# saitejasrivilli/movie-recommender-demo

Hardware: AMD Instinct MI355X
Metric: end-to-end recs/sec (1M ads d=256, top-500->10) (higher is better)
Workload: dtype f32 (f16x3 emulation: 2 fp16 planes per operand, 3 fp16-MFMA products per MAC, fp32 accumulate)

## Files before the change

movie-recommender-demo_amd/csrc/rowowner16_common.hpp:

```cpp
#pragma once
#include "x3_common.hpp"

namespace amdrec {
namespace x16 {

using x3::DBG, x3::f16x8, x3::lds_cfloat, x3::TARGET_EXP;

__device__ __forceinline__ f32x4 mfma(const f16x8& a, const f16x8& b, const f32x4& c) {
    return __builtin_amdgcn_mfma_f32_16x16x32_f16(a, b, c, 0, 0, 0);
}
__device__ __forceinline__ void group6(const f16x8 (&a)[4], const f16x8& bh, const f16x8& bl, f32x4& c0, f32x4& c1) {
    c0 = mfma(a[0], bl, c0);
    c1 = mfma(a[2], bl, c1);
    c0 = mfma(a[1], bh, c0);
    c1 = mfma(a[3], bh, c1);
    c0 = mfma(a[0], bh, c0);
    c1 = mfma(a[2], bh, c1);
}

__device__ __forceinline__ float reduce_max4(float v) {
    v = fmaxf(v, __shfl_xor(v, 16, 64));
    return fmaxf(v, __shfl_xor(v, 32, 64));
}
__device__ __forceinline__ float reduce_sum4(float v) {
    v += __shfl_xor(v, 16, 64);
    return v + __shfl_xor(v, 32, 64);
}

__device__ __forceinline__ void row_scale(const f32x4 (&x)[16], float& s, float& inv) {
    float m = 0.f;
#pragma unroll
    for (int t = 0; t < 16; ++t)
#pragma unroll
        for (int r = 0; r < 4; ++r) m = fmaxf(m, __builtin_fabsf(x[t][r]));
    m = reduce_max4(m);
    int eb = (int)((__float_as_uint(m) >> 23) & 0xffu);
    eb = eb < 87 ? 87 : (eb > 250 ? 250 : eb);
    s = __uint_as_float((uint32_t)(127 + TARGET_EXP + 127 - eb) << 23);
    inv = __uint_as_float((uint32_t)(eb - TARGET_EXP) << 23);
}

__device__ __forceinline__ void split8(const f32x4& a, const f32x4& b, float s, f16x8& h, f16x8& l) {
#pragma unroll
    for (int j = 0; j < 8; ++j) {
        const float v = (j < 4 ? a[j & 3] : b[j & 3]) * s;
        const _Float16 hh = (_Float16)v;
        h[j] = hh;
        l[j] = (_Float16)(v - (float)hh);
    }
}

__device__ __forceinline__ f32x4 param4(lds_cfloat* pb, int off, int tile) {
    return *reinterpret_cast<const __attribute__((address_space(3))) f32x4*>(pb + off + 16 * tile);
}

template <bool WITH_X>
__device__ __forceinline__ void prepare(const f32x4 (&x)[16], float s, lds_cfloat* pb, int bias, float scale,
                                        f16x8 (&xh)[8], f16x8 (&xl)[8], f32x4 (&acc)[16]) {
#pragma unroll
    for (int ks = 0; ks < 8; ++ks) {
        split8(x[2 * ks], x[2 * ks + 1], s, xh[ks], xl[ks]);
#pragma unroll
        for (int t = 2 * ks; t < 2 * ks + 2; ++t) {
            const f32x4 b = param4(pb, bias, t);
#pragma unroll
            for (int r = 0; r < 4; ++r) acc[t][r] = ((WITH_X ? x[t][r] : 0.f) + b[r]) * scale;
        }
    }
}

__device__ __forceinline__ float layer_norm(f32x4 (&y)[16], lds_cfloat* pb, int gamma, int beta, float eps) {
    float s = 0.f;
#pragma unroll
    for (int t = 0; t < 16; ++t)
#pragma unroll
        for (int r = 0; r < 4; ++r) s += y[t][r];
    const float mean = reduce_sum4(s) * (1.0f / 256.0f);
    float q = 0.f;
#pragma unroll
    for (int t = 0; t < 16; ++t)
#pragma unroll
        for (int r = 0; r < 4; ++r) {
            const float d = y[t][r] - mean;
            q += d * d;
        }
    const float rstd = 1.0f / sqrtf(reduce_sum4(q) * (1.0f / 256.0f) + eps);
#pragma unroll
    for (int t = 0; t < 16; ++t) {
        const f32x4 ga = param4(pb, gamma, t), be = param4(pb, beta, t);
#pragma unroll
        for (int r = 0; r < 4; ++r) y[t][r] = (y[t][r] - mean) * rstd * ga[r] + be[r];
    }
    return rstd;
}

__device__ __forceinline__ void layer_norm_scaled(const f32x4 (&acc)[16], float un, f32x4 (&y)[16], lds_cfloat* pb, int gamma,
                                                  int beta, float eps) {
    float s = 0.f;
#pragma unroll
    for (int t = 0; t < 16; ++t)
#pragma unroll
        for (int r = 0; r < 4; ++r) s += acc[t][r];
    const float mean = reduce_sum4(s) * un * (1.0f / 256.0f);
    float q = 0.f;
#pragma unroll
    for (int t = 0; t < 16; ++t)
#pragma unroll
        for (int r = 0; r < 4; ++r) {
            const float d = __builtin_fmaf(acc[t][r], un, -mean);
            y[t][r] = d;
            q += d * d;
        }
    const float rstd = 1.0f / sqrtf(reduce_sum4(q) * (1.0f / 256.0f) + eps);
#pragma unroll
    for (int t = 0; t < 16; ++t) {
        const f32x4 ga = param4(pb, gamma, t), be = param4(pb, beta, t);
#pragma unroll
        for (int r = 0; r < 4; ++r) y[t][r] = y[t][r] * rstd * ga[r] + be[r];
    }
}

__device__ __forceinline__ void hidden_planes(const f32x4& a0, const f32x4& a1, float c, float lim, f16x8& hh, f16x8& hl) {
    if (DBG & 8) {
        asm volatile("" : "+v"(hh), "+v"(hl) : "v"(a0), "v"(a1));
        return;
    }
    f32x4 t0, t1;
#pragma unroll
    for (int r = 0; r < 4; ++r) {
        t0[r] = __builtin_amdgcn_fmed3f(a0[r], 0.f, lim);
        t1[r] = __builtin_amdgcn_fmed3f(a1[r], 0.f, lim);
    }
    split8(t0, t1, c, hh, hl);
}
__device__ __forceinline__ void init_pair(f32x4& a0, f32x4& a1, lds_cfloat* pb, int bias, int tile0, float scale) {
    const f32x4 b0 = param4(pb, bias, tile0), b1 = param4(pb, bias, tile0 + 1);
#pragma unroll
    for (int r = 0; r < 4; ++r) {
        a0[r] = b0[r] * scale;
        a1[r] = b1[r] * scale;
    }
}

__device__ __forceinline__ void load_rows(f32x4 (&x)[16], const float* row_ptr, int g) {
#pragma unroll
    for (int t = 0; t < 16; ++t) x[t] = *reinterpret_cast<const f32x4*>(row_ptr + 16 * t + 4 * g);
}
__device__ __forceinline__ void add_rows(f32x4 (&x)[16], const float* row_ptr, int g) {
#pragma unroll
    for (int t = 0; t < 16; ++t) {
        const f32x4 v = *reinterpret_cast<const f32x4*>(row_ptr + 16 * t + 4 * g);
#pragma unroll
        for (int r = 0; r < 4; ++r) x[t][r] += v[r];
    }
}
__device__ __forceinline__ void store_rows(const f32x4 (&x)[16], float* row_ptr, int g) {
#pragma unroll
    for (int t = 0; t < 16; ++t) *reinterpret_cast<f32x4*>(row_ptr + 16 * t + 4 * g) = x[t];
}

}
}
```

movie-recommender-demo_amd/csrc/rowowner16_impl.hpp:

```cpp

#pragma clang diagnostic push
#pragma clang diagnostic ignored "-Wuninitialized-const-reference"
namespace amdrec {
namespace AMDREC_X3B_NAMESPACE {

using x3::CHUNK_BYTES, x3::CHUNK_FRAGS, x3::DBG, x3::f16x8, x3::FRAG_BYTES, x3::Input, x3::lds_byte, x3::lds_cfloat, x3::Phase,
    x3::Program, x3::RING_BYTES;
using x16::add_rows, x16::group6, x16::hidden_planes, x16::init_pair, x16::layer_norm, x16::layer_norm_scaled, x16::load_rows,
    x16::param4, x16::prepare, x16::reduce_sum4, x16::row_scale, x16::split8, x16::store_rows;

#if !defined(AMDREC_X3B_WAVES) || !defined(AMDREC_X3B_NAMESPACE)
#error "include rowowner16.hpp, not this file"
#endif
constexpr int WAVES = AMDREC_X3B_WAVES, ROWS_PER_WAVE = 16, ROWS_PER_WG = WAVES * ROWS_PER_WAVE;
constexpr int DMA_PER_WAVE = CHUNK_FRAGS / WAVES;
constexpr bool PAIRED = WAVES == 8 && !(DBG & (256 | 512));
constexpr int NBUF = PAIRED ? x3::NBUF - 1 : x3::NBUF, DEPTH = NBUF - 3;
constexpr int PAIR_BYTES = CHUNK_BYTES / 4;
constexpr int DMA_GROUP = 1;

struct Ring {
    lds_byte* lds_dma;
    lds_byte* lds_rd;
    int issued, total;
    int slot;
    __amdgpu_buffer_rsrc_t rsrc;
    uint32_t voff, soff0;
    const lds_byte* cbase;
    unsigned long long t_wait, t_bar, t_dma;
    unsigned long long t_lds, t_cal;
    __device__ __forceinline__ void timed_landed(f16x8 (&f)[4]) {
        if (!(DBG & 32)) return;
        const unsigned long long a = __builtin_amdgcn_s_memtime();
        asm volatile("s_waitcnt lgkmcnt(0)" : "+v"(f[0]), "+v"(f[1]), "+v"(f[2]), "+v"(f[3]));
        const unsigned long long b = __builtin_amdgcn_s_memtime();
        t_lds += b - a;
    }

    template <int U>
    __device__ __forceinline__ void dma_pieces(lds_byte* dst, uint32_t so) {
        if constexpr (U < DMA_PER_WAVE) {
            __builtin_amdgcn_raw_ptr_buffer_load_lds(rsrc, (__attribute__((address_space(3))) void*)(dst + (U >> 2) * 4 * FRAG_BYTES),
                                                     16, voff, so + (U >> 2) * 4 * FRAG_BYTES, (U & 3) * FRAG_BYTES, 0);
            dma_pieces<U + 1>(dst, so);
        }
    }
    __device__ __forceinline__ void issue() {
        if (DBG & 1) { ++issued; return; }
        const int c = issued < total ? issued : total - 1;
        lds_byte* dst = lds_dma + (uint32_t)(issued % NBUF) * CHUNK_BYTES;
        const uint32_t so = __builtin_amdgcn_readfirstlane(soff0 + (uint32_t)c * CHUNK_BYTES);
        dma_pieces<0>(dst, so);
        ++issued;
    }
    template <int EXTRA = 0>
    __device__ __forceinline__ void certify_next() {
        if (DBG & 16) {
            const unsigned long long a = __builtin_amdgcn_s_memtime();
            asm volatile("s_waitcnt vmcnt(%0)" ::"n"(DMA_PER_WAVE * (DEPTH - 1)) : "memory");
            const unsigned long long b = __builtin_amdgcn_s_memtime();
            __builtin_amdgcn_s_barrier();
            const unsigned long long c = __builtin_amdgcn_s_memtime();
            const unsigned long long d = __builtin_amdgcn_s_memtime();
            t_wait += b - a; t_bar += c - b; t_dma += d - c;
            return;
        }
        if (!(DBG & 1)) asm volatile("s_waitcnt vmcnt(%0)" ::"n"(DMA_PER_WAVE * (DEPTH - 1) + EXTRA) : "memory");
        if (!(DBG & 2)) __builtin_amdgcn_s_barrier();
    }
    __device__ __forceinline__ void start(const unsigned char* stream, int total_chunks, lds_byte* lds, int wave, int lane) {
        voff = (uint32_t)lane * 16;
        soff0 = (uint32_t)wave * DMA_PER_WAVE * FRAG_BYTES;
        rsrc = __builtin_amdgcn_make_buffer_rsrc(const_cast<unsigned char*>(stream), 0, (uint32_t)total_chunks * CHUNK_BYTES,
                                                 0x00020000);
        lds_dma = lds + wave * DMA_PER_WAVE * FRAG_BYTES;
        lds_rd = lds + lane * 16;
        issued = 0;
        total = total_chunks;
        slot = -1;
        cbase = lds_rd;
        t_wait = t_bar = t_dma = t_lds = 0;
        t_cal = 0;
        if (DBG & 32) {
            const unsigned long long a = __builtin_amdgcn_s_memtime();
            asm volatile("s_waitcnt lgkmcnt(0)" ::: "memory");
            const unsigned long long b = __builtin_amdgcn_s_memtime();
            t_cal = b - a;
        }
#pragma unroll
        for (int c = 0; c < DEPTH + 1; ++c) issue();
        asm volatile("s_waitcnt vmcnt(%0)" ::"n"(DMA_PER_WAVE * DEPTH) : "memory");
        __builtin_amdgcn_s_barrier();
    }
    template <int EXTRA = 0>
    __device__ __forceinline__ void advance() {
        certify_next<EXTRA>();
        slot = slot + 1 == NBUF ? 0 : slot + 1;
        cbase = lds_rd + (uint32_t)slot * CHUNK_BYTES;
    }
    template <int G, bool HALF = false>
    __device__ __forceinline__ void frag4(f16x8 (&f)[4]) {
        static_assert(G >= 0 && G < 4 && CHUNK_FRAGS == 16, "four groups of four fragment sets per chunk");
        if ((DBG & 4) || ((DBG & 64) && G != 0) || ((DBG & 128) && (G & 1)) ||
            (HALF && (DBG & (256 | 512)) && (G & 1))) {
#pragma unroll
            for (int u = 0; u < 4; ++u) asm volatile("" : "+v"(f[u]));
        } else {
#pragma unroll
            for (int u = 0; u < 4; ++u)
                f[u] = *reinterpret_cast<const __attribute__((address_space(3))) f16x8*>(cbase + (4 * G + u) * FRAG_BYTES);
        }
    }
    template <int G, int EXTRA = 0, bool HALF = false>
    __device__ __forceinline__ void read4(f16x8 (&f)[4]) {
        if (G == 0) advance<EXTRA>();
        frag4<G, HALF>(f);
        if (G == DMA_GROUP) issue();
    }
    __device__ __forceinline__ void drain() { asm volatile("s_waitcnt vmcnt(0)" ::: "memory"); }
};

template <int I>
__device__ __forceinline__ void gemm256_groups(Ring& ring, f16x8 (&cur)[4], const f16x8 (&xh)[8], const f16x8 (&xl)[8],
                                               f32x4 (&acc)[16]) {
    constexpr int ks = I >> 3, tp = I & 7;
    f16x8 nxt[4];
    if constexpr (I < 63) ring.read4<(I + 1) & 3>(nxt);
    ring.timed_landed(cur);
    group6(cur, xh[ks], xl[ks], acc[2 * tp], acc[2 * tp + 1]);
    if constexpr (I < 63) gemm256_groups<I + 1>(ring, nxt, xh, xl, acc);
}
template <int I0>
__device__ __forceinline__ void gemm256_from(Ring& ring, const f16x8 (&xh)[8], const f16x8 (&xl)[8], f32x4 (&acc)[16]) {
    f16x8 cur[4];
    ring.read4<0>(cur);
    gemm256_groups<I0>(ring, cur, xh, xl, acc);
}

__device__ __forceinline__ void gemm256(Ring& ring, const f16x8 (&xh)[8], const f16x8 (&xl)[8], f32x4 (&acc)[16]) {
    gemm256_from<0>(ring, xh, xl, acc);
}
__device__ __forceinline__ void phase_attn_ln(Ring& ring, const Phase& P, f32x4 (&x)[16], lds_cfloat* pb) {
    float s, inv;
    row_scale(x, s, inv);
    f16x8 xh[8], xl[8];
    f32x4 acc[16];
    prepare<true>(x, s, pb, P.b1, s * P.sw1, xh, xl, acc);
    gemm256(ring, xh, xl, acc);
    layer_norm_scaled(acc, inv / P.sw1, x, pb, P.gamma, P.beta, P.ln_eps);
}

template <bool S1, bool S2, int GI, int EXTRA = 0, bool HALF = false>
__device__ __forceinline__ void ffn_groups(Ring& ring, f16x8 (&cur)[4], const f16x8 (&xh)[8], const f16x8 (&xl)[8],
                                           f32x4& a10, f32x4& a11, f32x4 (&acc2)[16], const f16x8& hh, const f16x8& hl) {
    constexpr int NG = (S1 ? 8 : 0) + (S2 ? 8 : 0);
    constexpr bool is1 = S1 && (!S2 || (GI & 1) == 0);
    constexpr int u = (S1 && S2) ? GI >> 1 : GI;
    f16x8 nxt[4];
    if constexpr (GI < NG - 1) ring.read4<(GI + 1) & 3, EXTRA, HALF>(nxt);
    ring.timed_landed(cur);
    if constexpr (is1) group6(cur, xh[u], xl[u], a10, a11);
    else group6(cur, hh, hl, acc2[2 * u], acc2[2 * u + 1]);
    if constexpr (GI < NG - 1) ffn_groups<S1, S2, GI + 1, EXTRA, HALF>(ring, nxt, xh, xl, a10, a11, acc2, hh, hl);
}

template <bool S1, bool S2, int EXTRA = 0, bool HALF = false>
__device__ __forceinline__ void ffn_step(Ring& ring, const f16x8 (&xh)[8], const f16x8 (&xl)[8], f32x4& a10, f32x4& a11,
                                         f32x4 (&acc2)[16], const f16x8& hh, const f16x8& hl) {
    f16x8 cur[4];
    ring.read4<0, EXTRA, HALF>(cur);
    ffn_groups<S1, S2, 0, EXTRA, HALF>(ring, cur, xh, xl, a10, a11, acc2, hh, hl);
}

__device__ __forceinline__ void ffn_hidden(const f32x4& a0, const f32x4& a1, float c, float lim, f16x8& hh, f16x8& hl) {
    if (DBG & 512) asm volatile("" : "+v"(hh), "+v"(hl) : "v"(a0), "v"(a1));
    else hidden_planes(a0, a1, c, lim, hh, hl);
}
__device__ __forceinline__ void phase_ffn_ln(Ring& ring, const Phase& P, f32x4 (&x)[16], lds_cfloat* pb) {
    float s, inv;
    row_scale(x, s, inv);
    f16x8 xh[8], xl[8];
    const float sh = x3::hidden_scale(fmaf(P.hn * 8192.0f, inv, P.hb));
    f32x4 acc2[16];
    prepare<true>(x, s, pb, P.b2, P.sw2 * sh, xh, xl, acc2);
    const float b1s = s * P.sw1, c1 = sh * inv / P.sw1, lim1 = 60000.f / c1;
    f32x4 a10, a11;
    f16x8 hh, hl;
    init_pair(a10, a11, pb, P.b1, 0, b1s);
    ffn_step<true, false, 0, true>(ring, xh, xl, a10, a11, acc2, hh, hl);
    for (int t = 1; t < P.n_steps; ++t) {
        ffn_hidden(a10, a11, c1, lim1, hh, hl);
        init_pair(a10, a11, pb, P.b1, 2 * t, b1s);
        ffn_step<true, true, 0, true>(ring, xh, xl, a10, a11, acc2, hh, hl);
    }
    ffn_hidden(a10, a11, c1, lim1, hh, hl);
    ffn_step<false, true, 0, true>(ring, xh, xl, a10, a11, acc2, hh, hl);
    layer_norm_scaled(acc2, 1.0f / (P.sw2 * sh), x, pb, P.gamma, P.beta, P.ln_eps);
}

template <int K, class V>
__device__ __forceinline__ void pair_put(lds_byte* box, const V& v) {
    static_assert(sizeof(V) == 16 && K >= 0 && K < PAIR_BYTES / FRAG_BYTES, "a 16-byte piece per lane");
    *reinterpret_cast<__attribute__((address_space(3))) V*>(box + K * FRAG_BYTES) = v;
}
template <int K, class V>
__device__ __forceinline__ void pair_get(const lds_byte* box, V& v) {
    static_assert(sizeof(V) == 16 && K >= 0 && K < PAIR_BYTES / FRAG_BYTES, "a 16-byte piece per lane");
    v = *reinterpret_cast<const __attribute__((address_space(3))) V*>(box + K * FRAG_BYTES);
}
__device__ __forceinline__ void pair_landed() { asm volatile("s_waitcnt lgkmcnt(0)" ::: "memory"); }
__device__ __forceinline__ void pair_sync() {
    pair_landed();
    __builtin_amdgcn_s_barrier();
}
__device__ __forceinline__ void group12(const f16x8 (&a)[4], const f16x8& bh0, const f16x8& bl0, const f16x8& bh1,
                                        const f16x8& bl1, f32x4& c00, f32x4& c01, f32x4& c10, f32x4& c11) {
    c00 = x16::mfma(a[0], bl0, c00);
    c01 = x16::mfma(a[2], bl0, c01);
    c10 = x16::mfma(a[0], bl1, c10);
    c11 = x16::mfma(a[2], bl1, c11);
    c00 = x16::mfma(a[1], bh0, c00);
    c01 = x16::mfma(a[3], bh0, c01);
    c10 = x16::mfma(a[1], bh1, c10);
    c11 = x16::mfma(a[3], bh1, c11);
    c00 = x16::mfma(a[0], bh0, c00);
    c01 = x16::mfma(a[2], bh0, c01);
    c10 = x16::mfma(a[0], bh1, c10);
    c11 = x16::mfma(a[2], bh1, c11);
}
template <int MODE, int J>
__device__ __forceinline__ void pair_read(Ring& ring, f16x8 (&f)[4]) {
    constexpr int G = MODE == 0 ? (J & 3) : 2 * (J & 1) + (MODE == 2 ? 1 : 0);
    if constexpr (G == (MODE == 2 ? 1 : 0)) ring.advance();
    ring.frag4<G>(f);
    if constexpr (G == (MODE == 1 ? 2 : DMA_GROUP)) ring.issue();
}
template <int MODE, int J>
__device__ __forceinline__ void pair_groups1(Ring& ring, f16x8 (&cur)[4], const f16x8 (&xh)[2][8], const f16x8 (&xl)[2][8],
                                             f32x4 (&a)[2][2]) {
    f16x8 nxt[4];
    if constexpr (J < 7) pair_read<MODE, J + 1>(ring, nxt);
    ring.timed_landed(cur);
    group12(cur, xh[0][J], xl[0][J], xh[1][J], xl[1][J], a[0][0], a[0][1], a[1][0], a[1][1]);
    if constexpr (J < 7) pair_groups1<MODE, J + 1>(ring, nxt, xh, xl, a);
}
template <int MODE, int J>
__device__ __forceinline__ void pair_groups2(Ring& ring, f16x8 (&cur)[4], const f16x8 (&hh)[2], const f16x8 (&hl)[2],
                                             f32x4 (&acc2)[2][16]) {
    f16x8 nxt[4];
    if constexpr (J < 7) pair_read<MODE, J + 1>(ring, nxt);
    ring.timed_landed(cur);
    group12(cur, hh[0], hl[0], hh[1], hl[1], acc2[0][2 * J], acc2[0][2 * J + 1], acc2[1][2 * J], acc2[1][2 * J + 1]);
    if constexpr (J < 7) pair_groups2<MODE, J + 1>(ring, nxt, hh, hl, acc2);
}
__device__ __forceinline__ void pair_idle_step(Ring& ring) {
#pragma unroll
    for (int c = 0; c < 2; ++c) {
        ring.advance();
        ring.issue();
    }
}

__device__ __forceinline__ void pair_publish(const f32x4 (&a)[2][2], float c1, float lim1, lds_byte* box) {
    f16x8 hh, hl;
    hidden_planes(a[0][0], a[0][1], c1, lim1, hh, hl);
    pair_put<0>(box, hh);
    pair_put<1>(box, hl);
    pair_put<2>(box, a[1][0]);
    pair_put<3>(box, a[1][1]);
    pair_landed();
}
__device__ __forceinline__ void pair_fetch(const lds_byte* box, float c1, float lim1, f16x8 (&hh)[2], f16x8 (&hl)[2]) {
    f32x4 a0, a1;
    pair_get<0>(box, hh[0]);
    pair_get<1>(box, hl[0]);
    pair_get<2>(box, a0);
    pair_get<3>(box, a1);
    hidden_planes(a0, a1, c1, lim1, hh[1], hl[1]);
}

__device__ __forceinline__ void phase_ffn_ln_role_a(Ring& ring, const Phase& P, f32x4 (&x)[16], lds_cfloat* pb, lds_byte* box) {
    float s, inv;
    row_scale(x, s, inv);
    const float sh = x3::hidden_scale(fmaf(P.hn * 8192.0f, inv, P.hb));
    float b1s[2];
    b1s[0] = s * P.sw1;
    const float c1 = sh * inv / P.sw1, lim1 = 60000.f / c1;
    f16x8 xh[2][8], xl[2][8];
    {
        f32x4 acc2[16];
        prepare<true>(x, s, pb, P.b2, P.sw2 * sh, xh[0], xl[0], acc2);
        f32x4 sc = {P.sw2 * sh, 0.f, 0.f, 0.f};
        if (DBG & 1024) {
            sc[0] = b1s[0];
#pragma unroll
            for (int i = 0; i < 8; ++i) {
                asm volatile("" ::"v"(acc2[2 * i]), "v"(acc2[2 * i + 1]));
                xh[1][i] = xh[0][i], xl[1][i] = xl[0][i];
                asm volatile("" : "+v"(xh[1][i]), "+v"(xl[1][i]));
            }
        } else {
            pair_put<2>(box, sc);
            pair_sync();
            pair_get<0>(box, sc);
            pair_sync();
#pragma unroll
            for (int i = 0; i < 8; ++i) {
                pair_put<2>(box, acc2[2 * i]);
                pair_put<3>(box, acc2[2 * i + 1]);
                pair_sync();
                pair_get<0>(box, xh[1][i]);
                pair_get<1>(box, xl[1][i]);
                pair_sync();
            }
        }
        b1s[1] = sc[0];
    }
    f32x4 a[2][2];
    f16x8 cur[4];
    init_pair(a[0][0], a[0][1], pb, P.b1, 0, b1s[0]);
    init_pair(a[1][0], a[1][1], pb, P.b1, 0, b1s[1]);
    pair_read<0, 0>(ring, cur);
    pair_groups1<0, 0>(ring, cur, xh, xl, a);
    for (int t = 1; t < P.n_steps; ++t) {
        pair_publish(a, c1, lim1, box);
        init_pair(a[0][0], a[0][1], pb, P.b1, 2 * t, b1s[0]);
        init_pair(a[1][0], a[1][1], pb, P.b1, 2 * t, b1s[1]);
        pair_read<1, 0>(ring, cur);
        pair_groups1<1, 0>(ring, cur, xh, xl, a);
    }
    pair_publish(a, c1, lim1, box);
    pair_idle_step(ring);
#pragma unroll
    for (int k = 0; k < 4; ++k) {
        if (DBG & 1024) {
            asm volatile("" : "+v"(x[4 * k]), "+v"(x[4 * k + 1]), "+v"(x[4 * k + 2]), "+v"(x[4 * k + 3]));
            continue;
        }
        pair_sync();
        pair_get<0>(box, x[4 * k]);
        pair_get<1>(box, x[4 * k + 1]);
        pair_get<2>(box, x[4 * k + 2]);
        pair_get<3>(box, x[4 * k + 3]);
        pair_sync();
    }
}

__device__ __forceinline__ void phase_ffn_ln_role_b(Ring& ring, const Phase& P, f32x4 (&x)[16], lds_cfloat* pb, lds_byte* box) {
    float s, inv;
    row_scale(x, s, inv);
    const float sh = x3::hidden_scale(fmaf(P.hn * 8192.0f, inv, P.hb));
    float k2[2];
    k2[1] = P.sw2 * sh;
    const float c1 = sh * inv / P.sw1, lim1 = 60000.f / c1;
    f32x4 acc2[2][16];
    {
        f16x8 xh[8], xl[8];
        prepare<true>(x, s, pb, P.b2, k2[1], xh, xl, acc2[1]);
        f32x4 sc = {s * P.sw1, 0.f, 0.f, 0.f};
        if (DBG & 1024) {
            sc[0] = k2[1];
#pragma unroll
            for (int i = 0; i < 8; ++i) {
                asm volatile("" ::"v"(xh[i]), "v"(xl[i]));
                acc2[0][2 * i] = acc2[1][2 * i], acc2[0][2 * i + 1] = acc2[1][2 * i + 1];
                asm volatile("" : "+v"(acc2[0][2 * i]), "+v"(acc2[0][2 * i + 1]));
            }
        } else {
            pair_put<0>(box, sc);
            pair_sync();
            pair_get<2>(box, sc);
            pair_sync();
#pragma unroll
            for (int i = 0; i < 8; ++i) {
                pair_put<0>(box, xh[i]);
                pair_put<1>(box, xl[i]);
                pair_sync();
                pair_get<2>(box, acc2[0][2 * i]);
                pair_get<3>(box, acc2[0][2 * i + 1]);
                pair_sync();
            }
        }
        k2[0] = sc[0];
    }
    pair_idle_step(ring);
    f16x8 hh[2], hl[2], cur[4];
    for (int t = 1; t < P.n_steps; ++t) {
        pair_read<2, 0>(ring, cur);
        pair_fetch(box, c1, lim1, hh, hl);
        pair_groups2<2, 0>(ring, cur, hh, hl, acc2);
    }
    pair_read<0, 0>(ring, cur);
    pair_fetch(box, c1, lim1, hh, hl);
    pair_groups2<0, 0>(ring, cur, hh, hl, acc2);
    {
        f32x4 y[16];
        layer_norm_scaled(acc2[0], 1.0f / k2[0], y, pb, P.gamma, P.beta, P.ln_eps);
#pragma unroll
        for (int k = 0; k < 4; ++k) {
            if (DBG & 1024) {
                asm volatile("" ::"v"(y[4 * k]), "v"(y[4 * k + 1]), "v"(y[4 * k + 2]), "v"(y[4 * k + 3]));
                continue;
            }
            pair_put<0>(box, y[4 * k]);
            pair_put<1>(box, y[4 * k + 1]);
            pair_put<2>(box, y[4 * k + 2]);
            pair_put<3>(box, y[4 * k + 3]);
            pair_sync();
            pair_sync();
        }
    }
    layer_norm_scaled(acc2[1], 1.0f / k2[1], x, pb, P.gamma, P.beta, P.ln_eps);
}

struct HiddenRows {
    f32x4 p0, p1, q0, q1;
};
__device__ __forceinline__ void load_hidden(HiddenRows& h, const float* prow, const float* qrow, int t) {
    const float* pp = prow + 32 * t;
    const float* qq = qrow + 32 * t;
    asm volatile("global_load_dwordx4 %0, %4, off\n\t"
                 "global_load_dwordx4 %1, %4, off offset:64\n\t"
                 "global_load_dwordx4 %2, %5, off\n\t"
                 "global_load_dwordx4 %3, %5, off offset:64"
                 : "=&v"(h.p0), "=&v"(h.p1), "=&v"(h.q0), "=&v"(h.q1)
                 : "v"(pp), "v"(qq)
                 : "memory");
}
template <int N>
__device__ __forceinline__ void wait_hidden(HiddenRows& h) {
    asm volatile("s_waitcnt vmcnt(%4)" : "+v"(h.p0), "+v"(h.p1), "+v"(h.q0), "+v"(h.q1) : "n"(N) : "memory");
}
template <int EXTRA, int WAIT, bool LOAD>
__device__ __forceinline__ void cached_step(Ring& ring, const Phase& P, HiddenRows& h, const float* prow, const float* qrow,
                                            int t, float rstd, float sh, float lim, lds_cfloat* pb, f32x4 (&acc2)[16]) {
    const f32x4 c0 = param4(pb, P.b1, 2 * t), c1 = param4(pb, P.b1, 2 * t + 1);
    wait_hidden<WAIT>(h);
    f32x4 a0, a1;
#pragma unroll
    for (int r = 0; r < 4; ++r) {
        a0[r] = __builtin_fmaf(h.p0[r] + h.q0[r], rstd, c0[r]);
        a1[r] = __builtin_fmaf(h.p1[r] + h.q1[r], rstd, c1[r]);
    }
    f16x8 hh, hl, xh[8], xl[8];
    hidden_planes(a0, a1, sh, lim, hh, hl);
    if (LOAD) load_hidden(h, prow, qrow, t + 2);
    ffn_step<false, true, EXTRA>(ring, xh, xl, a0, a1, acc2, hh, hl);
}
__device__ __forceinline__ void phase_ffn_ln_cached(Ring& ring, const Phase& P, f32x4 (&x)[16], float rstd, const float* prow,
                                                    const float* qrow, lds_cfloat* pb) {
    HiddenRows ha, hb;
    load_hidden(ha, prow, qrow, 0);
    load_hidden(hb, prow, qrow, 1);
    float s, inv;
    row_scale(x, s, inv);
    const float sh = x3::hidden_scale(fmaf(P.hn * 8192.0f, inv, P.hb));
    const float k2 = P.sw2 * sh, lim = 60000.f / sh;
    f32x4 acc2[16];
#pragma unroll
    for (int t = 0; t < 16; ++t) {
        const f32x4 b = param4(pb, P.b2, t);
#pragma unroll
        for (int r = 0; r < 4; ++r) acc2[t][r] = (x[t][r] + b[r]) * k2;
    }
    const int T = P.n_steps;
    cached_step<8, 4, true>(ring, P, ha, prow, qrow, 0, rstd, sh, lim, pb, acc2);
    cached_step<8, 8, true>(ring, P, hb, prow, qrow, 1, rstd, sh, lim, pb, acc2);
    for (int t = 2; t < T - 2; t += 2) {
        cached_step<8, 12, true>(ring, P, ha, prow, qrow, t, rstd, sh, lim, pb, acc2);
        cached_step<8, 12, true>(ring, P, hb, prow, qrow, t + 1, rstd, sh, lim, pb, acc2);
    }
    cached_step<4, 12, false>(ring, P, ha, prow, qrow, T - 2, rstd, sh, lim, pb, acc2);
    cached_step<0, 8, false>(ring, P, hb, prow, qrow, T - 1, rstd, sh, lim, pb, acc2);
    layer_norm_scaled(acc2, 1.0f / k2, x, pb, P.gamma, P.beta, P.ln_eps);
}

template <int I>
__device__ __forceinline__ void cross_quarter_groups(Ring& ring, f16x8 (&cur)[4], const f16x8 (&xh)[8], const f16x8 (&xl)[8],
                                                     f32x4 (&acc)[4]) {
    constexpr int ks = I >> 1, pr = I & 1;
    f16x8 nxt[4];
    if constexpr (I < 15) ring.read4<(I + 1) & 3>(nxt);
    ring.timed_landed(cur);
    group6(cur, xh[ks], xl[ks], acc[2 * pr], acc[2 * pr + 1]);
    if constexpr (I < 15) cross_quarter_groups<I + 1>(ring, nxt, xh, xl, acc);
}

__device__ __forceinline__ void phase_cross(Ring& ring, const Phase& P, f32x4 (&xl_)[16], const f32x4 (&x0)[16], lds_cfloat* pb) {
    float s, inv;
    row_scale(xl_, s, inv);
    f16x8 xh[8], xl[8];
#pragma unroll
    for (int ks = 0; ks < 8; ++ks) split8(xl_[2 * ks], xl_[2 * ks + 1], s, xh[ks], xl[ks]);
    const float bs = s * P.sw1, un = inv / P.sw1;
#pragma unroll
    for (int q4 = 0; q4 < 4; ++q4) {
        f32x4 acc[4];
#pragma unroll
        for (int i = 0; i < 4; ++i) {
            const f32x4 b = param4(pb, P.b1, 4 * q4 + i);
#pragma unroll
            for (int r = 0; r < 4; ++r) acc[i][r] = b[r] * bs;
        }
        f16x8 cur[4];
        ring.read4<0>(cur);
        cross_quarter_groups<0>(ring, cur, xh, xl, acc);
#pragma unroll
        for (int i = 0; i < 4; ++i)
#pragma unroll
            for (int r = 0; r < 4; ++r) xl_[4 * q4 + i][r] = x0[4 * q4 + i][r] * (acc[i][r] * un) + xl_[4 * q4 + i][r];
    }
}

template <bool S1, bool S2, int P0, int GI>
__device__ __forceinline__ void heads_groups(Ring& ring, f16x8 (&cur)[4], const f16x8 (&xh)[8], const f16x8 (&xl)[8],
                                             f32x4& a10, f32x4& a11, f32x4 (&acc2)[4], const f16x8& hh, const f16x8& hl) {
    constexpr int NG = (S1 ? 8 : 0) + (S2 ? 2 : 0);
    constexpr bool is2 = S2 && (!S1 || GI == 4 || GI == 9);
    constexpr int u = !S1 ? 0 : (S2 ? (GI < 4 ? GI : GI - 1) : GI);
    constexpr int pr = !S1 ? GI : (GI == 9 ? 1 : 0);
    f16x8 nxt[4];
    if constexpr (GI < NG - 1) ring.read4<(P0 + GI + 1) & 3>(nxt);
    ring.timed_landed(cur);
    if constexpr (is2) group6(cur, hh, hl, acc2[2 * pr], acc2[2 * pr + 1]);
    else group6(cur, xh[u], xl[u], a10, a11);
    if constexpr (GI < NG - 1) heads_groups<S1, S2, P0, GI + 1>(ring, nxt, xh, xl, a10, a11, acc2, hh, hl);
}
template <bool S1, bool S2, int P0>
__device__ __forceinline__ void heads_step(Ring& ring, const f16x8 (&xh)[8], const f16x8 (&xl)[8], f32x4& a10, f32x4& a11,
                                           f32x4 (&acc2)[4], const f16x8& hh, const f16x8& hl) {
    f16x8 cur[4];
    ring.read4<P0>(cur);
    heads_groups<S1, S2, P0, 0>(ring, cur, xh, xl, a10, a11, acc2, hh, hl);
}

__device__ __forceinline__ void phase_heads(Ring& ring, const Program& G, const Phase& P, const f32x4 (&x)[16], float* out,
                                            long long ld_out, long long row, bool row_ok, int g, lds_cfloat* pb) {
    float s, inv;
    row_scale(x, s, inv);
    f16x8 xh[8], xl[8];
#pragma unroll
    for (int ks = 0; ks < 8; ++ks) split8(x[2 * ks], x[2 * ks + 1], s, xh[ks], xl[ks]);
    const float sh = x3::hidden_scale(fmaf(P.hn * 8192.0f, inv, P.hb));
    const float b1s = s * P.sw1, c1 = sh * inv / P.sw1, un2 = 1.0f / (P.sw2 * sh), lim1 = 60000.f / c1;
    const int T = P.n_steps, NT = P.n_tasks * T;
    f32x4 acc2[4], a10, a11;
    f16x8 hh, hl;
    init_pair(acc2[0], acc2[1], pb, G.hb2[0], 0, P.sw2 * sh);
    init_pair(acc2[2], acc2[3], pb, G.hb2[0], 2, P.sw2 * sh);
    init_pair(a10, a11, pb, P.b1, 0, b1s);
    heads_step<true, false, 0>(ring, xh, xl, a10, a11, acc2, hh, hl);
    const float probe = a10[0];
    int task = 0, t_in = 0;
    for (int tt = 1; tt <= NT; ++tt) {
        hidden_planes(a10, a11, c1, lim1, hh, hl);
        if (tt < NT) {
            init_pair(a10, a11, pb, P.b1, 2 * tt, b1s);
            if (tt & 1) heads_step<true, true, 0>(ring, xh, xl, a10, a11, acc2, hh, hl);
            else heads_step<true, true, 2>(ring, xh, xl, a10, a11, acc2, hh, hl);
        } else {
            heads_step<false, true, 2>(ring, xh, xl, a10, a11, acc2, hh, hl);
        }
        if (++t_in == T) {
            float dot = 0.f;
#pragma unroll
            for (int t = 0; t < 4; ++t) {
                const f32x4 w = param4(pb, G.hw3[task], t);
#pragma unroll
                for (int r = 0; r < 4; ++r) dot += fmaxf(acc2[t][r] * un2, 0.f) * w[r];
            }
            dot = reduce_sum4(dot);
            if (g == 0 && row_ok) out[(long long)task * ld_out + row] = x3::keep_nan(dot + pb[G.hb3[task]], probe);
            t_in = 0;
            if (++task < P.n_tasks) {
                init_pair(acc2[0], acc2[1], pb, G.hb2[task], 0, P.sw2 * sh);
                init_pair(acc2[2], acc2[3], pb, G.hb2[task], 2, P.sw2 * sh);
            }
        }
    }
}

__device__ __forceinline__ void run_chain(const Program& G, const Input& in, long long rows, float* scratch, float* x_out,
                                          long long ld_xout, float* logits, long long ld_logits, unsigned char* smem, int wave,
                                          int lane, lds_cfloat* pb) {
    const int g = lane >> 4, q = lane & 15;
    const long long row = (long long)blockIdx.x * ROWS_PER_WG + wave * ROWS_PER_WAVE + q;
    const bool row_ok = row < rows;
    const long long rowc = row_ok ? row : rows - 1;
    Ring ring;
    const unsigned long long t_begin = (DBG & 16) ? __builtin_amdgcn_s_memtime() : 0ull;
    ring.start(G.stream, G.total_chunks, (lds_byte*)smem, wave, lane);

    f32x4 x[16];
    if (in.X != nullptr) {
        load_rows(x, in.X + x3::dense_row(in, rowc) * in.ldx, g);
    } else {
        const long long gr = in.row_base + rowc;
        long long a = in.rowmap ? in.rowmap[gr] : gr;
        a = a < 0 ? 0 : (a >= in.n_cache ? in.n_cache - 1 : a);
        load_rows(x, in.cache + a * in.ldc, g);
        add_rows(x, in.U + (gr / in.rowdiv) * in.ldu, g);
    }
    int p = 0;
    float rstd = 0.f;
    for (; p < G.n_phases; ++p) {
        const Phase& P = G.ph[p];
        const int type = __builtin_amdgcn_readfirstlane(P.type);
        if (type == x3::PH_ATTN_LN) phase_attn_ln(ring, P, x, pb);
        else if (type == x3::PH_FFN_LN) {
            if constexpr (PAIRED) {
                lds_byte* box = (lds_byte*)smem + NBUF * CHUNK_BYTES + (wave & 3) * PAIR_BYTES + lane * 16;
                if (wave < 4) phase_ffn_ln_role_a(ring, P, x, pb, box);
                else phase_ffn_ln_role_b(ring, P, x, pb, box);
            } else {
                phase_ffn_ln(ring, P, x, pb);
            }
        }
        else if (type == x3::PH_LN) rstd = layer_norm(x, pb, P.gamma, P.beta, P.ln_eps);
        else if (WAVES == 8 && type == x3::PH_FFN_LN_CACHED) {
            if constexpr (WAVES == 8) {
                const long long gr = in.row_base + rowc;
                long long a = in.rowmap ? in.rowmap[gr] : gr;
                a = a < 0 ? 0 : (a >= in.n_cache ? in.n_cache - 1 : a);
                phase_ffn_ln_cached(ring, P, x, rstd, in.hcache + a * in.ldh + 4 * g, in.Q + (gr / in.rowdiv) * in.ldu + 4 * g,
                                    pb);
            }
        } else break;
    }
    if (p < G.n_phases && __builtin_amdgcn_readfirstlane(G.ph[p].type) == x3::PH_CROSS) {
        f32x4 x0[16];
#pragma unroll
        for (int t = 0; t < 16; ++t) x0[t] = x[t];
        for (; p < G.n_phases && __builtin_amdgcn_readfirstlane(G.ph[p].type) == x3::PH_CROSS; ++p)
            phase_cross(ring, G.ph[p], x, x0, pb);
    }
    if (p < G.n_phases) phase_heads(ring, G, G.ph[p], x, logits, ld_logits, row, row_ok, g, pb);
    if (x_out != nullptr && row_ok) store_rows(x, x_out + row * ld_xout, g);
    ring.drain();
    if ((DBG & 16) && lane == 0) {
        float* dbg = logits + 3 * ld_logits + ((long long)blockIdx.x * WAVES + wave) * 4;
        dbg[0] = (float)(__builtin_amdgcn_s_memtime() - t_begin);
        dbg[1] = (DBG & 32) ? (float)ring.t_lds : (float)ring.t_wait;
        dbg[2] = (DBG & 32) ? (float)ring.t_cal : (float)ring.t_bar;
        dbg[3] = (float)ring.t_dma;
    }
}

__global__ __launch_bounds__(64 * WAVES, 2) void ranker_x3b_kernel(Program G, Input in, long long rows, float* scratch,
                                                            float* x_out, long long ld_xout, float* logits,
                                                            long long ld_logits) {
    extern __shared__ __attribute__((aligned(16))) unsigned char smem[];
    const int tid = threadIdx.x, lane = tid & 63;
    const int wave = __builtin_amdgcn_readfirstlane(tid >> 6);
    const int g = lane >> 4;

    lds_byte* pbase = (lds_byte*)smem + RING_BYTES;
    for (int o = 0; o + wave * 1024 < G.n_params * 4; o += WAVES * 1024)
        __builtin_amdgcn_global_load_lds((const __attribute__((address_space(1))) void*)(
                                             reinterpret_cast<const unsigned char*>(G.params) + o + tid * 16),
                                         (__attribute__((address_space(3))) void*)(pbase + o + wave * 1024), 16, 0, 0);
    asm volatile("s_waitcnt vmcnt(0)" ::: "memory");
    lds_cfloat* pb = reinterpret_cast<lds_cfloat*>(pbase) + 4 * g;

    run_chain(G, in, rows, scratch, x_out, ld_xout, logits, ld_logits, smem, wave, lane, pb);
}

}
}
#pragma clang diagnostic pop
```

Measured before the change: 191,900.

## Overlap param, ring prefetch and row loads; hoist cached-hidden loads before first LN

```diff
diff --git a/movie-recommender-demo_amd/csrc/rowowner16_common.hpp b/movie-recommender-demo_amd/csrc/rowowner16_common.hpp
--- a/movie-recommender-demo_amd/csrc/rowowner16_common.hpp
+++ b/movie-recommender-demo_amd/csrc/rowowner16_common.hpp
@@ -154,6 +154,10 @@
         for (int r = 0; r < 4; ++r) x[t][r] += v[r];
     }
 }
+__device__ __forceinline__ void rows_landed(f32x4 (&x)[16]) {
+    asm volatile("" : "+v"(x[0]), "+v"(x[1]), "+v"(x[2]), "+v"(x[3]), "+v"(x[4]), "+v"(x[5]), "+v"(x[6]), "+v"(x[7]), "+v"(x[8]),
+                      "+v"(x[9]), "+v"(x[10]), "+v"(x[11]), "+v"(x[12]), "+v"(x[13]), "+v"(x[14]), "+v"(x[15]));
+}
 __device__ __forceinline__ void store_rows(const f32x4 (&x)[16], float* row_ptr, int g) {
 #pragma unroll
     for (int t = 0; t < 16; ++t) *reinterpret_cast<f32x4*>(row_ptr + 16 * t + 4 * g) = x[t];
diff --git a/movie-recommender-demo_amd/csrc/rowowner16_impl.hpp b/movie-recommender-demo_amd/csrc/rowowner16_impl.hpp
--- a/movie-recommender-demo_amd/csrc/rowowner16_impl.hpp
+++ b/movie-recommender-demo_amd/csrc/rowowner16_impl.hpp
@@ -68,7 +68,7 @@
         if (!(DBG & 1)) asm volatile("s_waitcnt vmcnt(%0)" ::"n"(DMA_PER_WAVE * (DEPTH - 1) + EXTRA) : "memory");
         if (!(DBG & 2)) __builtin_amdgcn_s_barrier();
     }
-    __device__ __forceinline__ void start(const unsigned char* stream, int total_chunks, lds_byte* lds, int wave, int lane) {
+    __device__ __forceinline__ void start_issue(const unsigned char* stream, int total_chunks, lds_byte* lds, int wave, int lane) {
         voff = (uint32_t)lane * 16;
         soff0 = (uint32_t)wave * DMA_PER_WAVE * FRAG_BYTES;
         rsrc = __builtin_amdgcn_make_buffer_rsrc(const_cast<unsigned char*>(stream), 0, (uint32_t)total_chunks * CHUNK_BYTES,
@@ -89,7 +89,9 @@
         }
 #pragma unroll
         for (int c = 0; c < DEPTH + 1; ++c) issue();
-        asm volatile("s_waitcnt vmcnt(%0)" ::"n"(DMA_PER_WAVE * DEPTH) : "memory");
+    }
+    __device__ __forceinline__ void start_wait() {
+        asm volatile("s_waitcnt vmcnt(%0)" ::"n"((DBG & 1) ? 0 : DMA_PER_WAVE * DEPTH) : "memory");
         __builtin_amdgcn_s_barrier();
     }
     template <int EXTRA = 0>
@@ -447,11 +449,8 @@
     if (LOAD) load_hidden(h, prow, qrow, t + 2);
     ffn_step<false, true, EXTRA>(ring, xh, xl, a0, a1, acc2, hh, hl);
 }
-__device__ __forceinline__ void phase_ffn_ln_cached(Ring& ring, const Phase& P, f32x4 (&x)[16], float rstd, const float* prow,
-                                                    const float* qrow, lds_cfloat* pb) {
-    HiddenRows ha, hb;
-    load_hidden(ha, prow, qrow, 0);
-    load_hidden(hb, prow, qrow, 1);
+__device__ __forceinline__ void phase_ffn_ln_cached(Ring& ring, const Phase& P, f32x4 (&x)[16], float rstd, HiddenRows& ha,
+                                                    HiddenRows& hb, const float* prow, const float* qrow, lds_cfloat* pb) {
     float s, inv;
     row_scale(x, s, inv);
     const float sh = x3::hidden_scale(fmaf(P.hn * 8192.0f, inv, P.hb));
@@ -582,27 +581,49 @@
 
 __device__ __forceinline__ void run_chain(const Program& G, const Input& in, long long rows, float* scratch, float* x_out,
                                           long long ld_xout, float* logits, long long ld_logits, unsigned char* smem, int wave,
-                                          int lane, lds_cfloat* pb) {
+                                          int lane) {
     const int g = lane >> 4, q = lane & 15;
     const long long row = (long long)blockIdx.x * ROWS_PER_WG + wave * ROWS_PER_WAVE + q;
     const bool row_ok = row < rows;
     const long long rowc = row_ok ? row : rows - 1;
+    const bool cached_head = WAVES == 8 && in.X == nullptr && G.n_phases >= 2 &&
+                             __builtin_amdgcn_readfirstlane(G.ph[0].type) == x3::PH_LN &&
+                             __builtin_amdgcn_readfirstlane(G.ph[1].type) == x3::PH_FFN_LN_CACHED;
+    const long long gr = in.row_base + rowc;
+    long long a = gr;
+    if (in.X == nullptr && in.rowmap != nullptr) a = in.rowmap[gr];
+    lds_byte* pbase = (lds_byte*)smem + RING_BYTES;
+    for (int o = 0; o + wave * 1024 < G.n_params * 4; o += WAVES * 1024)
+        __builtin_amdgcn_global_load_lds((const __attribute__((address_space(1))) void*)(
+                                             reinterpret_cast<const unsigned char*>(G.params) + o + (wave * 64 + lane) * 16),
+                                         (__attribute__((address_space(3))) void*)(pbase + o + wave * 1024), 16, 0, 0);
+    lds_cfloat* pb = reinterpret_cast<lds_cfloat*>(pbase) + 4 * g;
     Ring ring;
     const unsigned long long t_begin = (DBG & 16) ? __builtin_amdgcn_s_memtime() : 0ull;
-    ring.start(G.stream, G.total_chunks, (lds_byte*)smem, wave, lane);
-
     f32x4 x[16];
+    ring.start_issue(G.stream, G.total_chunks, (lds_byte*)smem, wave, lane);
     if (in.X != nullptr) {
         load_rows(x, in.X + x3::dense_row(in, rowc) * in.ldx, g);
     } else {
-        const long long gr = in.row_base + rowc;
-        long long a = in.rowmap ? in.rowmap[gr] : gr;
         a = a < 0 ? 0 : (a >= in.n_cache ? in.n_cache - 1 : a);
         load_rows(x, in.cache + a * in.ldc, g);
         add_rows(x, in.U + (gr / in.rowdiv) * in.ldu, g);
     }
+    ring.start_wait();
+    x16::rows_landed(x);
     int p = 0;
-    float rstd = 0.f;
+    if constexpr (WAVES == 8) {
+        if (cached_head) {
+            const float* prow = in.hcache + a * in.ldh + 4 * g;
+            const float* qrow = in.Q + (gr / in.rowdiv) * in.ldu + 4 * g;
+            HiddenRows ha, hb;
+            load_hidden(ha, prow, qrow, 0);
+            load_hidden(hb, prow, qrow, 1);
+            const float rstd = layer_norm(x, pb, G.ph[0].gamma, G.ph[0].beta, G.ph[0].ln_eps);
+            phase_ffn_ln_cached(ring, G.ph[1], x, rstd, ha, hb, prow, qrow, pb);
+            p = 2;
+        }
+    }
     for (; p < G.n_phases; ++p) {
         const Phase& P = G.ph[p];
         const int type = __builtin_amdgcn_readfirstlane(P.type);
@@ -616,16 +637,8 @@
                 phase_ffn_ln(ring, P, x, pb);
             }
         }
-        else if (type == x3::PH_LN) rstd = layer_norm(x, pb, P.gamma, P.beta, P.ln_eps);
-        else if (WAVES == 8 && type == x3::PH_FFN_LN_CACHED) {
-            if constexpr (WAVES == 8) {
-                const long long gr = in.row_base + rowc;
-                long long a = in.rowmap ? in.rowmap[gr] : gr;
-                a = a < 0 ? 0 : (a >= in.n_cache ? in.n_cache - 1 : a);
-                phase_ffn_ln_cached(ring, P, x, rstd, in.hcache + a * in.ldh + 4 * g, in.Q + (gr / in.rowdiv) * in.ldu + 4 * g,
-                                    pb);
-            }
-        } else break;
+        else if (type == x3::PH_LN) layer_norm(x, pb, P.gamma, P.beta, P.ln_eps);
+        else break;
     }
     if (p < G.n_phases && __builtin_amdgcn_readfirstlane(G.ph[p].type) == x3::PH_CROSS) {
         f32x4 x0[16];
@@ -652,17 +665,7 @@
     extern __shared__ __attribute__((aligned(16))) unsigned char smem[];
     const int tid = threadIdx.x, lane = tid & 63;
     const int wave = __builtin_amdgcn_readfirstlane(tid >> 6);
-    const int g = lane >> 4;
-
-    lds_byte* pbase = (lds_byte*)smem + RING_BYTES;
-    for (int o = 0; o + wave * 1024 < G.n_params * 4; o += WAVES * 1024)
-        __builtin_amdgcn_global_load_lds((const __attribute__((address_space(1))) void*)(
-                                             reinterpret_cast<const unsigned char*>(G.params) + o + tid * 16),
-                                         (__attribute__((address_space(3))) void*)(pbase + o + wave * 1024), 16, 0, 0);
-    asm volatile("s_waitcnt vmcnt(0)" ::: "memory");
-    lds_cfloat* pb = reinterpret_cast<lds_cfloat*>(pbase) + 4 * g;
-
-    run_chain(G, in, rows, scratch, x_out, ld_xout, logits, ld_logits, smem, wave, lane, pb);
+    run_chain(G, in, rows, scratch, x_out, ld_xout, logits, ld_logits, smem, wave, lane);
 }
 
 }
```

Result: no change. 192,800 (median of 6 runs) (+0.5%).
